# speechbrain/speechbrain

Measured on AMD Instinct MI355X. Metric: audio-sec/s decoded (node), Conformer-L beam=10, higher is better.
Workload: dtype f32

## Files before the change

speechbrain_amd/csrc/hip/sbk_device.h:

```cpp
#pragma once
#include <hip/hip_runtime.h>
#include <stdint.h>

namespace sbk {

constexpr int kWave = 64;

using f32x16 = __attribute__((ext_vector_type(16))) float;
using f32x4 = __attribute__((ext_vector_type(4))) float;

__device__ __forceinline__ f32x16 mfma_32x32x2(float a, float b, f32x16 acc) {
  return __builtin_amdgcn_mfma_f32_32x32x2f32(a, b, acc, 0, 0, 0);
}
__device__ __forceinline__ f32x4 mfma_16x16x4(float a, float b, f32x4 acc) {
  return __builtin_amdgcn_mfma_f32_16x16x4f32(a, b, acc, 0, 0, 0);
}

using bf16x8 = __attribute__((ext_vector_type(8))) __bf16;
__device__ __forceinline__ f32x16 mfma_32x32x16_bf16(bf16x8 a, bf16x8 b, f32x16 acc) {
  return __builtin_amdgcn_mfma_f32_32x32x16_bf16(a, b, acc, 0, 0, 0);
}
__device__ __forceinline__ unsigned short f32_to_bf16(float f) { return __builtin_bit_cast(unsigned short, (__bf16)f); }
__device__ __forceinline__ bf16x8 cvt_bf16x8(const float (&x)[8]) {
  bf16x8 r;
#pragma unroll
  for (int e = 0; e < 8; ++e) r[e] = (__bf16)x[e];
  return r;
}

using u32x4 = __attribute__((ext_vector_type(4))) unsigned;
__device__ __forceinline__ bf16x8 bf16x8_from_words(unsigned w0, unsigned w1, unsigned w2, unsigned w3) {
  u32x4 u = {w0, w1, w2, w3};
  return __builtin_bit_cast(bf16x8, u);
}
using bf16x2 = __attribute__((ext_vector_type(2))) __bf16;
__device__ __forceinline__ unsigned bf16_pair(float x0, float x1) {
  bf16x2 v = {(__bf16)x0, (__bf16)x1};
  return __builtin_bit_cast(unsigned, v);
}

using f16x8 = __attribute__((ext_vector_type(8))) _Float16;
__device__ __forceinline__ f32x16 mfma_32x32x16_f16(f16x8 a, f16x8 b, f32x16 acc) {
  return __builtin_amdgcn_mfma_f32_32x32x16_f16(a, b, acc, 0, 0, 0);
}
__device__ __forceinline__ unsigned short f32_to_f16(float f) { return __builtin_bit_cast(unsigned short, (_Float16)f); }
using fp8x8 = long;
__device__ __forceinline__ f32x16 mfma_32x32x16_fp8(fp8x8 a, fp8x8 b, f32x16 acc) {
  return __builtin_amdgcn_mfma_f32_32x32x16_fp8_fp8(a, b, acc, 0, 0, 0);
}
using i32x8 = __attribute__((ext_vector_type(8))) int;
__device__ __forceinline__ f32x16 mfma_32x32x64_fp8(i32x8 a, i32x8 b, f32x16 acc) {
  return __builtin_amdgcn_mfma_scale_f32_32x32x64_f8f6f4(a, b, acc, 0, 0, 0, 0, 0, 0);
}
__device__ __forceinline__ i32x8 i32x8_from_u4(uint4 lo, uint4 hi) {
  i32x8 r = {(int)lo.x, (int)lo.y, (int)lo.z, (int)lo.w, (int)hi.x, (int)hi.y, (int)hi.z, (int)hi.w};
  return r;
}
__device__ __forceinline__ unsigned short f32x2_to_fp8(float a, float b) {
  a = fminf(fmaxf(a, -448.0f), 448.0f);
  b = fminf(fmaxf(b, -448.0f), 448.0f);
  return (unsigned short)(__builtin_amdgcn_cvt_pk_fp8_f32(a, b, 0, false) & 0xffff);
}

using u16x8 = __attribute__((ext_vector_type(8))) unsigned short;
__device__ __forceinline__ bf16x8 pack_bf16x8(const unsigned short (&h)[8]) {
  u16x8 u;
#pragma unroll
  for (int e = 0; e < 8; ++e) u[e] = h[e];
  return __builtin_bit_cast(bf16x8, u);
}

__device__ __forceinline__ float shfl_xor(float v, int mask) { return __shfl_xor(v, mask, kWave); }
__device__ __forceinline__ int shfl_xor(int v, int mask) { return __shfl_xor(v, mask, kWave); }
__device__ __forceinline__ float shfl(float v, int lane) { return __shfl(v, lane, kWave); }
__device__ __forceinline__ int shfl(int v, int lane) { return __shfl(v, lane, kWave); }

__device__ __forceinline__ void wave_sync() { __builtin_amdgcn_wave_barrier(); }

__device__ __forceinline__ void sched_fence() { __builtin_amdgcn_sched_barrier(0); }

template <int MASK, int SIZE>
__device__ __forceinline__ void sched_group() { __builtin_amdgcn_sched_group_barrier(MASK, SIZE, 0); }

__device__ __forceinline__ void pin(unsigned& x) { asm volatile("" : "+v"(x)); }
__device__ __forceinline__ void pin(float& x) { asm volatile("" : "+v"(x)); }

__device__ __forceinline__ float exp2_raw(float x) { return __builtin_amdgcn_exp2f(x); }
__device__ __forceinline__ bool wave_any(bool p) { return __builtin_amdgcn_ballot_w64(p) != 0; }
__device__ __forceinline__ float gelu_erfc(float x) {
#pragma clang fp contract(off)
  const float z = fabsf(x) * 0.70710678118654752440f;
  const float t = __builtin_amdgcn_rcpf(fmaf(0.3275911f, z, 1.0f));
  float p = fmaf(t, 1.061405429f, -1.453152027f);
  p = fmaf(t, p, 1.421413741f);
  p = fmaf(t, p, -0.284496736f);
  p = fmaf(t, p, 0.254829592f);
  const float q = (p * t) * exp2_raw(-1.44269504088896340736f * (z * z));
  return (0.5f * x) * (x >= 0.0f ? 2.0f - q : q);
}

__device__ __forceinline__ float fast_ldexp(float x, int e) { return __builtin_amdgcn_ldexpf(x, e); }
__device__ __forceinline__ int frexp_exp(float x) { return __builtin_amdgcn_frexp_expf(x); }

template <int CTRL>
__device__ __forceinline__ float dpp_move(float v) {
  return __int_as_float(__builtin_amdgcn_update_dpp(0, __float_as_int(v), CTRL, 0xF, 0xF, true));
}
template <int G>
__device__ __forceinline__ float group_sum(float v) {
  static_assert(G == 1 || G == 2 || G == 4 || G == 8 || G == 16, "group_sum: group width");
  if constexpr (G >= 2) v += dpp_move<0xB1>(v);
  if constexpr (G >= 4) v += dpp_move<0x4E>(v);
  if constexpr (G >= 8) v += dpp_move<0x141>(v);
  if constexpr (G >= 16) v += dpp_move<0x140>(v);
  return v;
}


__device__ __forceinline__ void glds16(const float* src, float* lds_wave_base) {
  const unsigned dst = __builtin_amdgcn_readfirstlane(
      (unsigned)(unsigned long)(__attribute__((address_space(3))) void*)lds_wave_base);
  unsigned keep;
  asm volatile(
      "s_mov_b32 %0, m0\n\ts_mov_b32 m0, %2\n\ts_nop 0\n\tglobal_load_lds_dwordx4 %1, off\n\ts_mov_b32 m0, %0"
      : "=&s"(keep)
      : "v"(src), "s"(dst)
      : "memory");
}
__device__ __forceinline__ void glds16_uniform(const float* base, unsigned lane_byte_offset, float* lds_wave_base) {
  const unsigned dst = __builtin_amdgcn_readfirstlane(
      (unsigned)(unsigned long)(__attribute__((address_space(3))) void*)lds_wave_base);
  unsigned keep;
  asm volatile(
      "s_mov_b32 %0, m0\n\ts_mov_b32 m0, %3\n\ts_nop 0\n\tglobal_load_lds_dwordx4 %1, %2\n\ts_mov_b32 m0, %0"
      : "=&s"(keep)
      : "v"(lane_byte_offset), "s"(base), "s"(dst)
      : "memory");
}
template <bool NT>
__device__ __forceinline__ float4 ld16(const float* p) {
  if constexpr (NT) {
    const f32x4 v = __builtin_nontemporal_load(reinterpret_cast<const f32x4*>(p));
    return make_float4(v[0], v[1], v[2], v[3]);
  } else {
    return *reinterpret_cast<const float4*>(p);
  }
}
template <bool NT>
__device__ __forceinline__ float ld4(const float* p) {
  if constexpr (NT) return __builtin_nontemporal_load(p);
  else return *p;
}
__device__ __forceinline__ int uniform(int v) { return __builtin_amdgcn_readfirstlane(v); }
__device__ __forceinline__ void vm_drain() { asm volatile("s_waitcnt vmcnt(0)" ::: "memory"); }
__device__ __forceinline__ void vm_drain_visible() { __builtin_amdgcn_s_waitcnt(0x0F70); }
template <int N>
__device__ __forceinline__ void vm_wait() {
  static_assert(N >= 0 && N < 64, "vmcnt is a 6-bit counter");
  asm volatile("s_waitcnt vmcnt(%0)" ::"n"(N) : "memory");
}
__device__ __forceinline__ void lds_drain() { asm volatile("s_waitcnt lgkmcnt(0)" ::: "memory"); }
__device__ __forceinline__ void block_barrier_raw() { __builtin_amdgcn_s_barrier(); }
__device__ __forceinline__ void release_agent() {
  __builtin_amdgcn_fence(__ATOMIC_RELEASE, "agent");
  asm volatile("s_waitcnt vmcnt(0)" ::: "memory");
}
__device__ __forceinline__ void acquire_agent() { __builtin_amdgcn_fence(__ATOMIC_ACQUIRE, "agent"); }
__device__ __forceinline__ int atomic_add_agent(int* p, int v) {
// ... 111 lines not shown
```

speechbrain_amd/csrc/relpos_attn.hip:

```cpp
#include "common.h"
#include "internal.h"

namespace {

using sbk::f32x16;

struct AttnArgs {
  const float* qkv;
  const float* pos;
  const float* bias_u;
  const float* bias_v;
  const int32_t* key_len;
  float* out;
  float* attn;
  int B, T, H, SP;
  float scale;
  int chunk, left;
  int out_bf16;
};

__device__ __forceinline__ void key_range(const AttnArgs& a, int i, int klen, int& lo, int& hi) {
  lo = 0;
  hi = klen;
  if (a.chunk > 0) {
    const int c = i / a.chunk;
    hi = min((c + 1) * a.chunk, klen);
    if (a.left >= 0) lo = max(0, (c - a.left) * a.chunk);
  }
}

template <int N>
__device__ __forceinline__ void load_run(float (&dst)[N], const float* __restrict__ p) {
  if constexpr (N % 4 == 0) {
#pragma unroll
    for (int i = 0; i < N / 4; ++i) {
      const float4 v = reinterpret_cast<const float4*>(p)[i];
      dst[4 * i] = v.x; dst[4 * i + 1] = v.y; dst[4 * i + 2] = v.z; dst[4 * i + 3] = v.w;
    }
  } else if constexpr (N % 2 == 0) {
#pragma unroll
    for (int i = 0; i < N / 2; ++i) {
      const float2 v = reinterpret_cast<const float2*>(p)[i];
      dst[2 * i] = v.x; dst[2 * i + 1] = v.y;
    }
  } else {
#pragma unroll
    for (int i = 0; i < N; ++i) dst[i] = p[i];
  }
}

template <int DH, bool ROPE, bool PF, int NW>
__global__ void __launch_bounds__(NW * 64) relpos_attn_kernel(AttnArgs a) {
  constexpr int DH2 = DH / 2;
  constexpr int QP = DH + 1;
  constexpr int NC = (DH + 31) / 32;
  constexpr int NPART = NW / NC;
  constexpr int NT = NW * 64;
  SBK_DYN_LDS(float, lds);
  float* Qu = lds;
  float* Qv = Qu + 32 * QP;
  float* red = Qv + 32 * QP;
  float* S = red + (NW - NC) * 32 * 33;

  const int tid = threadIdx.x, lane = tid & 63, wave = tid >> 6;
  const int jl = lane & 31, half = lane >> 5;
  const int i0 = blockIdx.x * 32, h = blockIdx.y, b = blockIdx.z;
  const int T = a.T, SP = a.SP, d = a.H * DH;
  const size_t row3 = (size_t)3 * d;
  const float* qkv_b = a.qkv + (size_t)b * T * row3 + (size_t)h * 3 * DH;

  for (int idx = tid; idx < 32 * DH; idx += NT) {
    const int i = idx / DH, c = idx % DH;
    const int row = min(i0 + i, T - 1);
    const float q = qkv_b[(size_t)row * row3 + c];
    if constexpr (ROPE) {
      const float qs = qkv_b[(size_t)row * row3 + (c ^ 1)];
      Qu[i * QP + c] = (q * a.pos[(size_t)row * DH + c] + qs * a.bias_u[(size_t)row * DH + c]) * a.scale;
    } else {
      Qu[i * QP + c] = (q + a.bias_u[h * DH + c]) * a.scale;
      Qv[i * QP + c] = (q + a.bias_v[h * DH + c]) * a.scale;
    }
  }
// ... 318 lines not shown
  int kt_begin = 0, kt_end = nkt;
  if (a.chunk > 0) {
    kt_end = min(nkt, ((min(i0 + 31, T - 1) / a.chunk + 1) * a.chunk + 31) / 32);
    if (a.left >= 0) kt_begin = max(0, (i0 / a.chunk - a.left) * a.chunk) / 32;
  }
  float m_run = -INFINITY, l_run = 0.0f;
  f32x16 o[NC];
#pragma unroll
  for (int ct = 0; ct < NC; ++ct)
#pragma unroll
    for (int r = 0; r < 16; ++r) o[ct][r] = 0.0f;

  for (int kt = kt_begin; kt < kt_end; ++kt) {
    const int j0 = kt * 32;
    const int krow = min(j0 + jl, T - 1);
    f32x16 acc;
#pragma unroll
    for (int r = 0; r < 16; ++r) acc[r] = 0.0f;
#pragma unroll
    for (int p = 0; p < 2; ++p) {
      const int c0 = 64 * p + SEG * half;
      float kreg[SEG];
      load_run<SEG>(kreg, qkv_b + ((unsigned)krow * row3u + DH + c0));
      if (rot) rotate_chunks<SEG>(kreg, a.pos + (size_t)krow * DH + c0, a.bias_u + (size_t)krow * DH + c0);
#pragma unroll
      for (int s = 0; s < SEG; ++s) acc = sbk::mfma_32x32x2(kreg[s], qu[p][s], acc);
      sbk::sched_fence();
    }
    auto load_v = [&](int ct, float (&vv)[16]) {
      unsigned t0 = j0 + 4 * half;
      sbk::pin(t0);
#pragma unroll
      for (int r = 0; r < 16; ++r) {
        const unsigned t = min(t0 + (r & 3) + 8 * (r >> 2), (unsigned)(T - 1));
        vv[r] = qkv_b[t * row3u + (2 * DH + ct * 32 + jl)];
      }
    };
    float vv[2][16];
    load_v(0, vv[0]);
    float mx = -INFINITY;
#pragma unroll
    for (int r = 0; r < 16; ++r) {
      const int key = j0 + (r & 3) + 8 * (r >> 2) + 4 * half;
      if (!(key >= lo && key < hi)) acc[r] = -INFINITY;
      mx = fmaxf(mx, acc[r]);
    }
    mx = fmaxf(mx, sbk::shfl_xor(mx, 32));
    const float m_new = fmaxf(m_run, mx);
    const float alpha = m_new == -INFINITY ? 1.0f : expf(m_run - m_new);
    float sum = 0.0f;
#pragma unroll
    for (int r = 0; r < 16; ++r) {
      acc[r] = acc[r] == -INFINITY ? 0.0f : expf(acc[r] - m_new);
      sum += acc[r];
    }
    sum += sbk::shfl_xor(sum, 32);
    l_run = l_run * alpha + sum;
    m_run = m_new;
    if (sbk::wave_any(alpha != 1.0f)) {
#pragma unroll
      for (int ct = 0; ct < NC; ++ct)
#pragma unroll
        for (int r = 0; r < 16; ++r) o[ct][r] *= alpha;
    }
#pragma unroll
    for (int ct = 0; ct < NC; ++ct) {
      if (ct + 1 < NC) load_v(ct + 1, vv[(ct + 1) & 1]);
#pragma unroll
      for (int r = 0; r < 16; ++r) o[ct] = sbk::mfma_32x32x2(vv[ct & 1][r], acc[r], o[ct]);
    }
  }
  if (i0 + jl < T) {
    const float inv = l_run > 0.0f ? 1.0f / l_run : 0.0f;
    float* orow = a.out + ((size_t)b * T + i0 + jl) * d + h * DH;
#pragma unroll
    for (int ct = 0; ct < NC; ++ct)
#pragma unroll
      for (int q = 0; q < 4; ++q)
        *reinterpret_cast<float4*>(orow + ct * 32 + 8 * q + 4 * half) =
            make_float4(o[ct][4 * q] * inv, o[ct][4 * q + 1] * inv, o[ct][4 * q + 2] * inv, o[ct][4 * q + 3] * inv);
  }
}

template <int DH, bool E2 = true>
__global__ void __launch_bounds__(256, 2) relpos_flash_t_kernel(AttnArgs a) {
  constexpr int DH2 = DH / 2;
  constexpr int NC = (DH + 31) / 32;
  __shared__ float Gs[4][64][32];
  const int tid = threadIdx.x, lane = tid & 63, wave = tid >> 6;
  const int jl = lane & 31, half = lane >> 5;
  const int i0 = (blockIdx.x * 4 + wave) * 32, h = blockIdx.y, b = blockIdx.z;
  const int T = a.T, d = a.H * DH;
  if (i0 >= T) return;
  const size_t row3 = (size_t)3 * d;
  const float* qkv_b = a.qkv + (size_t)b * T * row3 + (size_t)h * 3 * DH;
  const int qrow = min(i0 + jl, T - 1);
  float (*G)[32] = Gs[wave];

  float qu[DH2], qv[DH2];
  {
    float qr[DH2], bu[DH2], bv[DH2];
    load_run<DH2>(qr, qkv_b + (size_t)qrow * row3 + half * DH2);
    load_run<DH2>(bu, a.bias_u + h * DH + half * DH2);
    load_run<DH2>(bv, a.bias_v + h * DH + half * DH2);
#pragma unroll
    for (int s = 0; s < DH2; ++s) {
      qu[s] = (qr[s] + bu[s]) * a.scale;
      qv[s] = (qr[s] + bv[s]) * a.scale;
    }
  }
  int klen = T;
  if (a.key_len) klen = min(max(a.key_len[b], 1), T);
  const int nkt = (klen + 31) / 32;
  int lo, hi;
  key_range(a, qrow, klen, lo, hi);
  int kt_begin = 0, kt_end = nkt;
  if (a.chunk > 0) {
    kt_end = min(nkt, ((min(i0 + 31, T - 1) / a.chunk + 1) * a.chunk + 31) / 32);
    if (a.left >= 0) kt_begin = max(0, (i0 / a.chunk - a.left) * a.chunk) / 32;
  }
  float m_run = -INFINITY, l_run = 0.0f;
  f32x16 o[NC];
#pragma unroll
  for (int ct = 0; ct < NC; ++ct)
#pragma unroll
    for (int r = 0; r < 16; ++r) o[ct][r] = 0.0f;

  auto g_block = [&](int first_row, int slot) {
    float preg[DH2];
    const int prow = min(max(first_row + jl, 0), 2 * T - 2);
    load_run<DH2>(preg, a.pos + (size_t)prow * d + h * DH + half * DH2);
    f32x16 g;
#pragma unroll
    for (int r = 0; r < 16; ++r) g[r] = 0.0f;
#pragma unroll
    for (int s = 0; s < DH2; ++s) g = sbk::mfma_32x32x2(preg[s], qv[s], g);
#pragma unroll
    for (int r = 0; r < 16; ++r) G[slot * 32 + (r & 3) + 8 * (r >> 2) + 4 * half][jl] = g[r];
  };
  g_block((T - 1) - i0 - 31 + 32 * kt_begin, kt_begin & 1);
  for (int kt = kt_begin; kt < kt_end; ++kt) {
    const int j0 = kt * 32;
    const int rbase = (T - 1) - i0 - 31 + j0;
    float kreg[DH2];
    load_run<DH2>(kreg, qkv_b + (size_t)min(j0 + jl, T - 1) * row3 + DH + half * DH2);
    f32x16 acc;
#pragma unroll
    for (int r = 0; r < 16; ++r) acc[r] = 0.0f;
#pragma unroll
    for (int s = 0; s < DH2; ++s) acc = sbk::mfma_32x32x2(kreg[s], qu[s], acc);
    g_block(rbase + 32, (kt + 1) & 1);
    float vv[NC][16];
#pragma unroll
    for (int ct = 0; ct < NC; ++ct) {
      const int col = ct * 32 + jl;
      const float* vbase = qkv_b + 2 * DH + (col < DH ? col : 0);
#pragma unroll
      for (int r = 0; r < 16; ++r) {
        const int t = min(j0 + (r & 3) + 8 * (r >> 2) + 4 * half, T - 1);
        vv[ct][r] = col < DH ? vbase[(size_t)t * row3] : 0.0f;
      }
    }
    sbk::wave_sync();
    float mx = -INFINITY;
#pragma unroll
    for (int r = 0; r < 16; ++r) {
      const int jc = (r & 3) + 8 * (r >> 2) + 4 * half;
      const int rr = 31 - jl + jc;
      acc[r] += G[(((kt & 1) + (rr >> 5)) & 1) * 32 + (rr & 31)][jl];
      const int key = j0 + jc;
      if (!(key >= lo && key < hi)) acc[r] = -INFINITY;
      mx = fmaxf(mx, acc[r]);
    }
    sbk::wave_sync();
    mx = fmaxf(mx, sbk::shfl_xor(mx, 32));
    const float m_new = fmaxf(m_run, mx);
    constexpr float kL2E = 1.44269504088896340736f;
    const bool none = m_new == -INFINITY;
    const float nm = none ? 0.0f : -m_new * kL2E;
    float alpha, sum = 0.0f;
    if constexpr (E2) {
      alpha = none ? 1.0f : sbk::exp2_raw(fmaf(m_run, kL2E, nm));
#pragma unroll
      for (int r = 0; r < 16; ++r) {
        acc[r] = none ? 0.0f : sbk::exp2_raw(fmaf(acc[r], kL2E, nm));
        sum += acc[r];
      }
    } else {
      alpha = none ? 1.0f : expf(m_run - m_new);
#pragma unroll
      for (int r = 0; r < 16; ++r) {
        acc[r] = acc[r] == -INFINITY ? 0.0f : expf(acc[r] - m_new);
        sum += acc[r];
      }
    }
    sum += sbk::shfl_xor(sum, 32);
    l_run = l_run * alpha + sum;
    m_run = m_new;
    if (sbk::wave_any(alpha != 1.0f)) {
#pragma unroll
      for (int ct = 0; ct < NC; ++ct)
#pragma unroll
        for (int r = 0; r < 16; ++r) o[ct][r] *= alpha;
    }
#pragma unroll
    for (int r = 0; r < 16; ++r)
#pragma unroll
      for (int ct = 0; ct < NC; ++ct) o[ct] = sbk::mfma_32x32x2(vv[ct][r], acc[r], o[ct]);
  }
  if (i0 + jl < T) {
    const float inv = l_run > 0.0f ? 1.0f / l_run : 0.0f;
    float* orow = a.out + ((size_t)b * T + i0 + jl) * d + h * DH;
#pragma unroll
    for (int ct = 0; ct < NC; ++ct)
#pragma unroll
      for (int r = 0; r < 16; ++r) {
        const int c = ct * 32 + (r & 3) + 8 * (r >> 2) + 4 * half;
        if (c < DH) orow[c] = o[ct][r] * inv;
      }
  }
}

__global__ void __launch_bounds__(256, 2) rope_flash_t_bf16_kernel(AttnArgs a) {
  constexpr int DH = 64;
  using sbk::bf16x8;
  const int tid = threadIdx.x, lane = tid & 63, wave = tid >> 6;
  const int jl = lane & 31, half = lane >> 5;
  const int i0 = (blockIdx.x * 4 + wave) * 32, h = blockIdx.y, b = blockIdx.z;
  const int T = a.T, d = a.H * DH;
  if (i0 >= T) return;
  const size_t row3 = (size_t)3 * d;
  const float* qkv_b = a.qkv + (size_t)b * T * row3 + (size_t)h * 3 * DH;
  const int qrow = min(i0 + jl, T - 1);

  auto load_chunks = [&](const float* row, int frame, float scale, bf16x8 (&dst)[4]) {
#pragma unroll
    for (int t = 0; t < 4; ++t) {
      const int c0 = 16 * t + 8 * half;
      float x[8];
      load_run<8>(x, row + c0);
      if (a.pos != nullptr) {
        float cs[8], sn[8];
        load_run<8>(cs, a.pos + (size_t)frame * DH + c0);
        load_run<8>(sn, a.bias_u + (size_t)frame * DH + c0);
#pragma unroll
        for (int e = 0; e < 8; e += 2) {
          const float x0 = x[e], x1 = x[e + 1];
          x[e] = x0 * cs[e] + x1 * sn[e];
          x[e + 1] = x1 * cs[e + 1] + x0 * sn[e + 1];
        }
      }
#pragma unroll
      for (int e = 0; e < 8; ++e) x[e] *= scale;
      dst[t] = sbk::cvt_bf16x8(x);
    }
  };
  bf16x8 qb[4];
  load_chunks(qkv_b + (size_t)qrow * row3, qrow, a.scale, qb);

  int klen = T;
  if (a.key_len) klen = min(max(a.key_len[b], 1), T);
  const int nkt = (klen + 31) / 32;
  int lo, hi;
  key_range(a, qrow, klen, lo, hi);
  int kt_begin = 0, kt_end = nkt;
  if (a.chunk > 0) {
    kt_end = min(nkt, ((min(i0 + 31, T - 1) / a.chunk + 1) * a.chunk + 31) / 32);
    if (a.left >= 0) kt_begin = max(0, (i0 / a.chunk - a.left) * a.chunk) / 32;
  }
  float m_run = -INFINITY, l_run = 0.0f;
  f32x16 o[2];
#pragma unroll
  for (int ct = 0; ct < 2; ++ct)
#pragma unroll
    for (int r = 0; r < 16; ++r) o[ct][r] = 0.0f;

  for (int kt = kt_begin; kt < kt_end; ++kt) {
    const int j0 = kt * 32;
    bf16x8 kb[4];
    {
      const int krow = min(j0 + jl, T - 1);
      load_chunks(qkv_b + (size_t)krow * row3 + DH, krow, 1.0f, kb);
    }
    f32x16 acc;
#pragma unroll
    for (int r = 0; r < 16; ++r) acc[r] = 0.0f;
#pragma unroll
    for (int t = 0; t < 4; ++t) acc = sbk::mfma_32x32x16_bf16(kb[t], qb[t], acc);
    bf16x8 vb[2][2];
#pragma unroll
    for (int ct = 0; ct < 2; ++ct) {
// ... 155 lines not shown
        acc[u] = sbk::mfma_32x32x16_bf16(kb, qb[t], acc[u]);
      }
    }
    float mx = -INFINITY;
    const bool tail = (kt + 1) * 64 > klen;
    if (tail) {
#pragma unroll
      for (int u = 0; u < 2; ++u)
#pragma unroll
        for (int r = 0; r < 16; ++r)
          if (kt * 64 + 32 * u + 16 * (r >> 3) + 8 * half + (r & 7) >= klen) acc[u][r] = -INFINITY;
    }
#pragma unroll
    for (int u = 0; u < 2; ++u)
#pragma unroll
      for (int r = 0; r < 16; ++r) mx = fmaxf(mx, acc[u][r]);
    mx = fmaxf(mx, sbk::shfl_xor(mx, 32));
    const float m_new = fmaxf(m_run, mx);
    const float c2 = a.scale * 1.44269504088896340736f, mc = -m_new * c2;
    const float alpha = sbk::exp2_raw((m_run - m_new) * c2);
    float sum = 0.0f;
    bf16x8 pb[2][2];
#pragma unroll
    for (int u = 0; u < 2; ++u)
#pragma unroll
      for (int s2 = 0; s2 < 2; ++s2) {
        float x[8];
#pragma unroll
        for (int e = 0; e < 8; ++e) {
          x[e] = sbk::exp2_raw(fmaf(acc[u][8 * s2 + e], c2, mc));
          sum += x[e];
        }
        pb[u][s2] = sbk::cvt_bf16x8(x);
      }
    sum += sbk::shfl_xor(sum, 32);
    l_run = l_run * alpha + sum;
    m_run = m_new;
    if (sbk::wave_any(alpha != 1.0f)) {
#pragma unroll
      for (int c = 0; c < 2; ++c)
#pragma unroll
        for (int r = 0; r < 16; ++r) o[c][r] *= alpha;
    }
#pragma unroll
    for (int u = 0; u < 2; ++u)
#pragma unroll
      for (int s2 = 0; s2 < 2; ++s2)
#pragma unroll
        for (int c = 0; c < 2; ++c) {
          const bf16x8 vb = *reinterpret_cast<const bf16x8*>(Vt + (32 * c + jl) * 32 + (((4 * u + 2 * s2 + half) ^ vsw) << 2));
          o[c] = sbk::mfma_32x32x16_bf16(vb, pb[u][s2], o[c]);
        }
    sbk::vm_drain();
    __syncthreads();
  }
  if (i0 + jl < T) {
    const float inv = 1.0f / l_run;
    unsigned short* orow = a.out + ((size_t)b * T + i0 + jl) * d + h * 64;
#pragma unroll
    for (int c = 0; c < 2; ++c)
#pragma unroll
      for (int q = 0; q < 4; ++q) {
        uint2 pk;
        pk.x = (unsigned)sbk::f32_to_bf16(o[c][4 * q] * inv) | ((unsigned)sbk::f32_to_bf16(o[c][4 * q + 1] * inv) << 16);
        pk.y = (unsigned)sbk::f32_to_bf16(o[c][4 * q + 2] * inv) | ((unsigned)sbk::f32_to_bf16(o[c][4 * q + 3] * inv) << 16);
        *reinterpret_cast<uint2*>(orow + c * 32 + 8 * q + 4 * half) = pk;
      }
  }
}

}
namespace sbk {
int g_attn_exp2 = 1;
}
namespace {
template <int DH, bool ROPE>
int launch_flash(const AttnArgs& a, hipStream_t st) {
  sbk::ProfScope prof(ROPE ? "rope_attention" : "relpos_attention", (ROPE ? 4.0 : 6.0) * a.B * a.H * (double)a.T * a.T * DH,
                      4.0 * a.B * a.T * (4.0 * a.H * DH) + 4.0 * (2.0 * a.T - 1) * a.H * DH, st);
  if constexpr (ROPE) {
    SBK_LAUNCH((rope_flash_t_kernel<DH>), dim3((a.T + 127) / 128, a.H, a.B), dim3(256), 0, st, a);
    return sbk::launch_status("sbk_rope_attention_f32");
  } else {
    if (sbk::g_attn_exp2) {
      SBK_LAUNCH((relpos_flash_t_kernel<DH, true>), dim3((a.T + 127) / 128, a.H, a.B), dim3(256), 0, st, a);
    } else {
      SBK_LAUNCH((relpos_flash_t_kernel<DH, false>), dim3((a.T + 127) / 128, a.H, a.B), dim3(256), 0, st, a);
    }
    return sbk::launch_status("sbk_relpos_attention_f32");
  }
}

int launch_flash128(const AttnArgs& a, hipStream_t st) {
  if (a.attn)
    return sbk::fail(SBK_EINVAL, "rope_attention: the attention-weights output is not instantiated for head_dim 128 (context only)");
  if ((double)a.T * 3.0 * a.H * 128 >= 1073741824.0)
    return sbk::fail(SBK_EINVAL, "rope_attention: head_dim 128 addresses an utterance's rows with 32-bit offsets: T * 3 * d must be < 2^30");
  if (!sbk::aligned16(a.out)) return sbk::fail(SBK_EINVAL, "rope_attention: head_dim 128 writes 16-byte pieces: out must be 16-byte aligned");
  sbk::ProfScope prof("rope_attention", 4.0 * a.B * a.H * (double)a.T * a.T * 128, 4.0 * a.B * a.T * (4.0 * a.H * 128), st);
  SBK_LAUNCH(rope_flash_t128_kernel, dim3((a.T + 127) / 128, a.H, a.B), dim3(256), 0, st, a);
  return sbk::launch_status("sbk_rope_attention_f32");
}

template <int DH, bool ROPE, bool PF, int NW>
int launch_attn_pf(const AttnArgs& a, hipStream_t st);

template <int DH, bool ROPE>
int launch_attn(const AttnArgs& a, hipStream_t st) {
  if (!a.attn) return launch_flash<DH, ROPE>(a, st);
  const size_t lds4 = ((size_t)2 * 32 * (DH + 1) + 3 * 32 * 33 + (size_t)32 * a.SP) * sizeof(float);
  const bool eight = lds4 > 80 * 1024;
  const bool pf = ROPE && eight;
  if (eight) return pf ? launch_attn_pf<DH, ROPE, true, 8>(a, st) : launch_attn_pf<DH, ROPE, false, 8>(a, st);
  return pf ? launch_attn_pf<DH, ROPE, true, 4>(a, st) : launch_attn_pf<DH, ROPE, false, 4>(a, st);
}

template <int DH, bool ROPE, bool PF, int NW>
int launch_attn_pf(const AttnArgs& a, hipStream_t st) {
  constexpr int NCt = (DH + 31) / 32;
  const size_t lds = ((size_t)2 * 32 * (DH + 1) + (NW - NCt) * 32 * 33 + (size_t)32 * a.SP) * sizeof(float);
  if (lds > 160 * 1024) return sbk::fail(SBK_EINVAL, "relpos_attention: T=%d needs %zu B of LDS (max 160 KiB)", a.T, lds);
  if (const int rc = sbk::require_dyn_lds(relpos_attn_kernel<DH, ROPE, PF, NW>, lds, "relpos_attention")) return rc;
  sbk::ProfScope prof(ROPE ? "rope_attention" : "relpos_attention", (ROPE ? 4.0 : 6.0) * a.B * a.H * (double)a.T * a.T * DH,
                      4.0 * a.B * a.T * (4.0 * a.H * DH) + 4.0 * (2.0 * a.T - 1) * a.H * DH, st);
  SBK_LAUNCH((relpos_attn_kernel<DH, ROPE, PF, NW>), dim3((a.T + 31) / 32, a.H, a.B), dim3(NW * 64), lds, st, a);
  return sbk::launch_status(ROPE ? "sbk_rope_attention_f32" : "sbk_relpos_attention_f32");
}

}

namespace sbk {

int relpos_attention(const float* qkv, const float* pos, const float* bias_u, const float* bias_v,
                     const int32_t* key_len, float* out, float* attn, int B, int T, int H, int Dh, float scale,
                     hipStream_t st, int chunk, int left) {
  if (B == 0 || T == 0) return 0;
  const int SP = ((T + 31) / 32) * 32 + 1;
  AttnArgs a{qkv, pos, bias_u, bias_v, key_len, out, attn, B, T, H, SP, scale, chunk, left};
  switch (Dh) {
    case 64: return launch_attn<64, false>(a, st);
    case 36: return launch_attn<36, false>(a, st);
    case 32: return launch_attn<32, false>(a, st);
    case 16: return launch_attn<16, false>(a, st);
    case 8: return launch_attn<8, false>(a, st);
    default: return fail(SBK_EINVAL, "relpos_attention: head_dim %d not instantiated (8,16,32,36,64)", Dh);
  }
}

int rope_attention(const float* qkv, const float* cosines, const float* sines, const int32_t* key_len, float* out,
                   float* attn, int B, int T, int H, int Dh, float scale, hipStream_t st, int chunk, int left) {
  if (B == 0 || T == 0) return 0;
  const int SP = ((T + 31) / 32) * 32 + 1;
  AttnArgs a{qkv, cosines, sines, nullptr, key_len, out, attn, B, T, H, SP, scale, chunk, left};
  switch (Dh) {
    case 128: return launch_flash128(a, st);
    case 64: return launch_attn<64, true>(a, st);
    case 36: return launch_attn<36, true>(a, st);
    case 32: return launch_attn<32, true>(a, st);
    case 16: return launch_attn<16, true>(a, st);
    case 8: return launch_attn<8, true>(a, st);
    default: return fail(SBK_EINVAL, "rope_attention: head_dim %d not instantiated (8,16,32,36,64,128)", Dh);
  }
}
}

extern "C" int sbk_rope_attention_f32(const float* qkv, const float* cosines, const float* sines,
                                      const int32_t* key_len, float* out, float* attn, int B, int T, int H, int Dh,
                                      int table_rows, float scale, int chunk_size, int left_chunks,
                                      sbk_stream_t stream) {
  if (B == 0 || T == 0) return 0;
// ... 81 lines not shown
```

speechbrain_amd/native.py:

```python

from __future__ import annotations

import collections
import contextlib
import ctypes
import math
import os
import threading
import weakref
from ctypes import POINTER, c_char_p, c_float, c_int, c_int32, c_void_p
from typing import Optional

import torch

_HERE = os.path.dirname(os.path.abspath(__file__))
LIB_PATH = os.path.join(_HERE, "csrc", "libsbk_hip.so")

ACT_NONE, ACT_SWISH, ACT_GELU, ACT_RELU, ACT_LEAKY_RELU = 0, 1, 2, 3, 4

_lib = None


class SbkError(RuntimeError):
    pass
# ... 161 lines not shown
        "sbk_w2v_utt_norm_f32": ([p, p, i, ctypes.c_long, f, p], c_int),
        "sbk_wavlm_attention_max_frames": ([], c_int),
        "sbk_wavlm_attention_f32": ([p, p, p, p, p, p, p, p, i, i, i, i, f, p], c_int),
        "sbk_hypermix_split_frames": ([], c_int),
        "sbk_hypermix_workspace_bytes": ([i, i, i, i], ctypes.c_size_t),
        "sbk_hypermix_f32": ([p] * 13 + [f, p, p, p, ctypes.c_size_t, i, i, i, i, i, p], c_int),
        "sbk_rnn_layer_route": ([i, i, i, i], c_int),
        "sbk_rnn_layer_f32": ([p] * 9 + [i] * 6 + [p], c_int),
        "sbk_crdnn_conv1_f32": ([p] * 6 + [i, i, i, i, f, f, p], c_int),
        "sbk_crdnn_im2col_f32": ([p, p, i, i, i, i, i, i, p], c_int),
        "sbk_crdnn_norm_pool_f32": ([p] * 4 + [i] * 6 + [f, f, p], c_int),
        "sbk_layernorm_f32": ([p, p, p, p, i, i, f, i, p], c_int),
        "sbk_log_softmax_f32": ([p, p, i, i, f, f, p], c_int),
        "sbk_ctc_greedy_decode_f32": ([p, p, p, p, i, i, i, i, p], c_int),
        "sbk_ctc_beam_search_workspace_bytes": ([i, i, i, i, i], ctypes.c_size_t),
        "sbk_ctc_beam_search_f32": ([p, p, p, i, POINTER(CTCBeamConfig), p, ctypes.c_size_t, p, p, p, i, i, i, p], c_int),
        "sbk_ctc_beam_search_lm_f32": ([p, p, p, i, POINTER(CTCBeamConfig), POINTER(CTCLMTables), p, ctypes.c_size_t, p, p, p,
                                        p, i, i, i, p], c_int),
        "sbk_transducer_greedy_f32": ([POINTER(TransducerWeights), POINTER(TransducerConfig), p, p, p, p, p, p, p, i, i, p],
                                      c_int),
        "sbk_lstm_f32": ([p, p, p, p, p, p, p, i, i, i, p], c_int),
        "sbk_transducer_beam_workspace_bytes": ([POINTER(TransducerWeights), POINTER(TransducerBeamConfig), i, i],
                                                ctypes.c_size_t),
        "sbk_transducer_beam_search_f32": ([POINTER(TransducerWeights), POINTER(TransducerBeamConfig), p, p, ctypes.c_size_t,
                                            p, p, p, p, p, i, i, p], c_int),
        "sbk_transducer_beam_lm_workspace_bytes": ([POINTER(TransducerWeights), POINTER(RNNLMWeights),
                                                    POINTER(TransducerBeamConfig), i, i], ctypes.c_size_t),
        "sbk_transducer_beam_search_lm_f32": ([POINTER(TransducerWeights), POINTER(RNNLMWeights), f,
                                               POINTER(TransducerBeamConfig), p, p, ctypes.c_size_t, p, p, p, p, p, i, i, p],
                                              c_int),
        "sbk_beam_search_workspace_bytes": ([POINTER(DecoderWeights), POINTER(SearchConfig), i, i], ctypes.c_size_t),
        "sbk_beam_search_f32": ([POINTER(DecoderWeights), POINTER(SearchConfig), p, p, p, p, p, ctypes.c_size_t, p, p,
                                 p, p, p, p, p, POINTER(c_int32), i, i, p], c_int),
        "sbk_greedy_search_workspace_bytes": ([POINTER(DecoderWeights), i, i, i], ctypes.c_size_t),
        "sbk_greedy_search_f32": ([POINTER(DecoderWeights), p, p, p, ctypes.c_size_t, p, p, p, POINTER(c_int32), i, i,
                                   i, i, i, i, i, p], c_int),
        "sbk_prompted_greedy_search_workspace_bytes": ([POINTER(DecoderWeights), i, i, i, i], ctypes.c_size_t),
        "sbk_prompted_greedy_search_f32": ([POINTER(DecoderWeights), p, p, p, i, p, p, p, ctypes.c_size_t, p, p, i, i, p, p,
                                            POINTER(c_int32), i, i, i, i, i, p], c_int),
        "sbk_decoder_prefix_workspace_bytes": ([POINTER(DecoderWeights), i, i, i], ctypes.c_size_t),
        "sbk_decoder_prefix_f32": ([POINTER(DecoderWeights), p, p, p, p, ctypes.c_size_t, p, i, i, i, p], c_int),
        "sbk_lm_prefix_workspace_bytes": ([POINTER(LMWeights), i, i], ctypes.c_size_t),
        "sbk_lm_prefix_f32": ([POINTER(LMWeights), p, p, ctypes.c_size_t, p, i, i, p], c_int),
    }
    for name, (args, res) in sig.items():
        fn = getattr(lib, name)
        fn.argtypes = args
        fn.restype = res
    return sig


EXPORTS: tuple = ()
_LIBS: dict = {}


def load(path: Optional[str] = None):
    global _lib, EXPORTS
    if _lib is not None and path is None:
        return _lib
    path = path or LIB_PATH
    if path not in _LIBS:
        if not os.path.exists(path):
            raise SbkError(
                f"{path} is missing: the MI355X kernels are not built. Run `python -m speechbrain_amd.csrc.build` "
                "(hipcc, gfx950). There is no CPU fallback."
            )
        lib = ctypes.CDLL(path)
        exports = tuple(_declare(lib).keys())
        if lib.sbk_abi_version() != 11:
            raise SbkError(f"ABI version mismatch: {lib.sbk_abi_version()}")
        _LIBS[path] = (lib, exports)
    _lib, EXPORTS = _LIBS[path]
    return _lib


KNOBS = {
    "skinny_off": 2, "cross_rows": 4, "cross_fc256": 8, "tiled_splitk": 14, "sk_mode": 18, "sk_min_rows": 24,
    "x3_route_rows": 34, "x3_route_tiles": 35, "score_fused": 40, "x3r_mode": 41, "x3r_min_rows": 42, "x3r_ln": 45,
    "persist": 47, "persist_grid": 48, "persist_stamps": 49, "x3r_xc": 51, "nt_mask": 53, "self_anc": 55, "x3r_pair": 58,
    "persist_tree": 59, "attn_exp2": 60, "lp256": 61, "x3p_fast_epi": 63,
}


@contextlib.contextmanager
def knobs(**values):
    lib = load()
    wanted = {KNOBS[name]: int(value) for name, value in values.items()}
    found = {key: lib.sbk_prof_get_knob(key) for key in wanted}
    try:
        for key, value in wanted.items():
            lib.sbk_prof_set_knob(key, value)
        yield
    finally:
        for key, value in found.items():
            lib.sbk_prof_set_knob(key, value)


def _chk(rc: int, what: str):
    if rc != 0:
        raise SbkError(f"{what} failed (rc={rc}): {_lib.sbk_last_error().decode()}")


def _dev_ok(*ts):
    for t in ts:
        if t is None:
            continue
        if not t.is_cuda:
            raise SbkError(
                "speechbrain_amd ops run on an MI355X (HIP) device only; got a CPU tensor. "
                "Move the module and inputs to 'cuda' (there is no CPU fallback)."
            )
        if not t.is_contiguous():
            raise SbkError("non-contiguous tensor passed to a kernel")


def _p(t: Optional[torch.Tensor]):
    return None if t is None else c_void_p(t.data_ptr())


_STREAM_WS = {}
_STREAM_WS_LOCK = threading.RLock()
_STREAM_WS_REFS = {}


def _ws_key(stream):
    return (id(load()), stream.device.index, stream.cuda_stream) if stream is not None else (id(load()), "host", 0)


def retain_stream_workspace(stream):
    key = _ws_key(stream)
    with _STREAM_WS_LOCK:
        _STREAM_WS_REFS[key] = _STREAM_WS_REFS.get(key, 0) + 1


class _Workspace:
    __slots__ = ("buf", "off", "ptr", "key")

    def __init__(self, nbytes, device, align=256, floor=0, per_stream=False):
        size = max(nbytes, floor) + align
        self.buf, self.key = (_search_workspace(size, device) if per_stream
                              else (torch.empty(size, dtype=torch.uint8, device=device), None))
        self.off = (-self.buf.data_ptr()) % align
        self.ptr = c_void_p(self.buf.data_ptr() + self.off)

    def __enter__(self):
        return self

    def __exit__(self, *exc):
        _search_workspace_done(self.key)


def _register_workspace(key, device, handle):
    lib = load()
    with _STREAM_WS_LOCK:
        if key in _STREAM_WS:
            return
        nbytes = lib.sbk_stream_workspace_bytes()
        ws = _Workspace(nbytes, device)
        ctx = torch.cuda.device(device) if getattr(device, "type", None) == "cuda" else contextlib.nullcontext()
        with ctx:
            _chk(lib.sbk_stream_workspace_set(c_void_p(handle) if handle is not None else None, ws.ptr, nbytes),
                 "sbk_stream_workspace_set")
        _STREAM_WS[key] = ws


def forget_stream_owner(stream):
    key = _ws_key(stream)
    with _STREAM_WS_LOCK:
        left = _STREAM_WS_REFS.get(key, 0) - 1
        if left > 0:
            _STREAM_WS_REFS[key] = left
# ... 1615 lines not shown
```

Before: 13140.

## Prefetch next K and position rows one tile ahead in relpos flash attention

Restructures the relpos flash-attention tile loop so the K and positional-embedding rows for the next key tile are loaded while the current tile computes. The loop is software-pipelined with scheduling fences and register pins. It also switches address arithmetic to 32-bit offsets and simplifies the G-ring index and the key-mask comparisons, which cuts per-element integer work. The new path is on by default, guarded by a size check, and can be disabled through a bit in the attn_exp2 knob. The cost is extra register pressure from double-buffered K and P registers, which could hurt occupancy at launch bounds of 256 threads with 2 blocks.

New measurement: 13250, median of 6. About the same (+0.8%).

```diff
diff --git a/speechbrain_amd/csrc/hip/sbk_device.h b/speechbrain_amd/csrc/hip/sbk_device.h
--- a/speechbrain_amd/csrc/hip/sbk_device.h
+++ b/speechbrain_amd/csrc/hip/sbk_device.h
@@ -84,6 +84,7 @@
 
 __device__ __forceinline__ void pin(unsigned& x) { asm volatile("" : "+v"(x)); }
 __device__ __forceinline__ void pin(float& x) { asm volatile("" : "+v"(x)); }
+__device__ __forceinline__ void pin(f32x4& x) { asm volatile("" : "+v"(x)); }
 
 __device__ __forceinline__ float exp2_raw(float x) { return __builtin_amdgcn_exp2f(x); }
 __device__ __forceinline__ bool wave_any(bool p) { return __builtin_amdgcn_ballot_w64(p) != 0; }
diff --git a/speechbrain_amd/csrc/relpos_attn.hip b/speechbrain_amd/csrc/relpos_attn.hip
--- a/speechbrain_amd/csrc/relpos_attn.hip
+++ b/speechbrain_amd/csrc/relpos_attn.hip
@@ -1,3 +1,5 @@
+#include <type_traits>
+
 #include "common.h"
 #include "internal.h"
 
@@ -482,12 +484,31 @@
   }
 }
 
-template <int DH, bool E2 = true>
+__device__ __forceinline__ const float* at32(const float* base, unsigned elem) {
+  return reinterpret_cast<const float*>(reinterpret_cast<const char*>(base) + elem * 4u);
+}
+template <int N>
+__device__ __forceinline__ void pin_run(float (&x)[N]) {
+  if constexpr (N % 4 == 0) {
+#pragma unroll
+    for (int i = 0; i < N / 4; ++i) {
+      sbk::f32x4 t;
+      t[0] = x[4 * i]; t[1] = x[4 * i + 1]; t[2] = x[4 * i + 2]; t[3] = x[4 * i + 3];
+      sbk::pin(t);
+      x[4 * i] = t[0]; x[4 * i + 1] = t[1]; x[4 * i + 2] = t[2]; x[4 * i + 3] = t[3];
+    }
+  } else {
+#pragma unroll
+    for (int s = 0; s < N; ++s) sbk::pin(x[s]);
+  }
+}
+
+template <int DH, bool E2 = true, bool AH = true>
 __global__ void __launch_bounds__(256, 2) relpos_flash_t_kernel(AttnArgs a) {
   constexpr int DH2 = DH / 2;
   constexpr int NC = (DH + 31) / 32;
   __shared__ float Gs[4][64][32];
-  const int tid = threadIdx.x, lane = tid & 63, wave = tid >> 6;
+  const int tid = threadIdx.x, lane = tid & 63, wave = AH ? sbk::uniform(tid >> 6) : tid >> 6;
   const int jl = lane & 31, half = lane >> 5;
   const int i0 = (blockIdx.x * 4 + wave) * 32, h = blockIdx.y, b = blockIdx.z;
   const int T = a.T, d = a.H * DH;
@@ -526,10 +547,44 @@
 #pragma unroll
     for (int r = 0; r < 16; ++r) o[ct][r] = 0.0f;
 
-  auto g_block = [&](int first_row, int slot) {
-    float preg[DH2];
+  float kreg[DH2], preg[DH2], vv[NC][16];
+  const unsigned row3u = 3u * (unsigned)d;
+  auto k_req = [&](int kt) SBK_INLINE_LAMBDA {
+    if constexpr (AH) load_run<DH2>(kreg, at32(qkv_b, (unsigned)min(kt * 32 + jl, T - 1) * row3u + (unsigned)(DH + half * DH2)));
+    else load_run<DH2>(kreg, qkv_b + (size_t)min(kt * 32 + jl, T - 1) * row3 + DH + half * DH2);
+  };
+  auto p_req = [&](int first_row) SBK_INLINE_LAMBDA {
     const int prow = min(max(first_row + jl, 0), 2 * T - 2);
-    load_run<DH2>(preg, a.pos + (size_t)prow * d + h * DH + half * DH2);
+    if constexpr (AH) load_run<DH2>(preg, at32(a.pos + h * DH, (unsigned)prow * (unsigned)d + (unsigned)(half * DH2)));
+    else load_run<DH2>(preg, a.pos + (size_t)prow * d + h * DH + half * DH2);
+  };
+  auto v_req = [&](int kt) SBK_INLINE_LAMBDA {
+    if constexpr (AH) {
+#pragma unroll
+      for (int r = 0; r < 16; ++r) {
+        const int t = min(kt * 32 + (r & 3) + 8 * (r >> 2) + 4 * half, T - 1);
+#pragma unroll
+        for (int ct = 0; ct < NC; ++ct) {
+          const int col = ct * 32 + jl;
+          vv[ct][r] = col < DH ? *at32(qkv_b + 2 * DH, (unsigned)t * row3u + (unsigned)(col < DH ? col : 0)) : 0.0f;
+        }
+        sbk::sched_fence();
+      }
+    } else {
+#pragma unroll
+      for (int ct = 0; ct < NC; ++ct) {
+        const int col = ct * 32 + jl;
+        const float* vbase = qkv_b + 2 * DH + (col < DH ? col : 0);
+#pragma unroll
+        for (int r = 0; r < 16; ++r) {
+          const int t = min(kt * 32 + (r & 3) + 8 * (r >> 2) + 4 * half, T - 1);
+          vv[ct][r] = col < DH ? vbase[(size_t)t * row3] : 0.0f;
+        }
+      }
+    }
+  };
+  auto g_chain = [&](int slot) SBK_INLINE_LAMBDA {
+    if constexpr (AH) pin_run(preg);
     f32x16 g;
 #pragma unroll
     for (int r = 0; r < 16; ++r) g[r] = 0.0f;
@@ -538,38 +593,65 @@
 #pragma unroll
     for (int r = 0; r < 16; ++r) G[slot * 32 + (r & 3) + 8 * (r >> 2) + 4 * half][jl] = g[r];
   };
-  g_block((T - 1) - i0 - 31 + 32 * kt_begin, kt_begin & 1);
-  for (int kt = kt_begin; kt < kt_end; ++kt) {
+  const int first = (T - 1) - i0 - 31 + 32 * kt_begin;
+  if constexpr (AH) {
+    if (kt_begin < kt_end) {
+      p_req(first);
+      k_req(kt_begin);
+      sbk::sched_fence();
+      g_chain(kt_begin & 1);
+      sbk::sched_fence();
+      p_req(first + 32);
+      sbk::sched_fence();
+    }
+  } else {
+    p_req(first);
+    g_chain(kt_begin & 1);
+  }
+  auto tile = [&](int kt, auto more_c) SBK_INLINE_LAMBDA {
+    constexpr bool MORE = decltype(more_c)::value;
     const int j0 = kt * 32;
     const int rbase = (T - 1) - i0 - 31 + j0;
-    float kreg[DH2];
-    load_run<DH2>(kreg, qkv_b + (size_t)min(j0 + jl, T - 1) * row3 + DH + half * DH2);
+    if constexpr (AH) pin_run(kreg);
+    else k_req(kt);
     f32x16 acc;
 #pragma unroll
     for (int r = 0; r < 16; ++r) acc[r] = 0.0f;
 #pragma unroll
     for (int s = 0; s < DH2; ++s) acc = sbk::mfma_32x32x2(kreg[s], qu[s], acc);
-    g_block(rbase + 32, (kt + 1) & 1);
-    float vv[NC][16];
-#pragma unroll
-    for (int ct = 0; ct < NC; ++ct) {
-      const int col = ct * 32 + jl;
-      const float* vbase = qkv_b + 2 * DH + (col < DH ? col : 0);
-#pragma unroll
-      for (int r = 0; r < 16; ++r) {
-        const int t = min(j0 + (r & 3) + 8 * (r >> 2) + 4 * half, T - 1);
-        vv[ct][r] = col < DH ? vbase[(size_t)t * row3] : 0.0f;
-      }
+    if constexpr (AH) {
+      sbk::sched_fence();
+      if constexpr (MORE) k_req(kt + 1);
+      v_req(kt);
+      sbk::sched_fence();
+    } else {
+      p_req(rbase + 32);
+    }
+    g_chain((kt + 1) & 1);
+    if constexpr (AH) {
+      sbk::sched_fence();
+      if constexpr (MORE) p_req(rbase + 64);
+      sbk::sched_fence();
+    } else {
+      v_req(kt);
     }
     sbk::wave_sync();
     float mx = -INFINITY;
+    unsigned ring0 = (unsigned)((kt & 1) * 32 + 31 - jl + 4 * half);
+    if constexpr (AH) sbk::pin(ring0);
+    const int klo = lo - (j0 + 4 * half), khi = hi - (j0 + 4 * half);
 #pragma unroll
     for (int r = 0; r < 16; ++r) {
       const int jc = (r & 3) + 8 * (r >> 2) + 4 * half;
       const int rr = 31 - jl + jc;
-      acc[r] += G[(((kt & 1) + (rr >> 5)) & 1) * 32 + (rr & 31)][jl];
+      if constexpr (AH) acc[r] += G[(ring0 + (r & 3) + 8 * (r >> 2)) & 63][jl];
+      else acc[r] += G[(((kt & 1) + (rr >> 5)) & 1) * 32 + (rr & 31)][jl];
       const int key = j0 + jc;
-      if (!(key >= lo && key < hi)) acc[r] = -INFINITY;
+      if constexpr (AH) {
+        if (!((r & 3) + 8 * (r >> 2) >= klo && (r & 3) + 8 * (r >> 2) < khi)) acc[r] = -INFINITY;
+      } else {
+        if (!(key >= lo && key < hi)) acc[r] = -INFINITY;
+      }
       mx = fmaxf(mx, acc[r]);
     }
     sbk::wave_sync();
@@ -603,10 +685,25 @@
 #pragma unroll
         for (int r = 0; r < 16; ++r) o[ct][r] *= alpha;
     }
+    if constexpr (AH) {
+#pragma unroll
+      for (int ct = 0; ct < NC; ++ct)
+#pragma unroll
+        for (int r = 0; r < 16; ++r) sbk::pin(vv[ct][r]);
+    }
 #pragma unroll
     for (int r = 0; r < 16; ++r)
 #pragma unroll
       for (int ct = 0; ct < NC; ++ct) o[ct] = sbk::mfma_32x32x2(vv[ct][r], acc[r], o[ct]);
+  };
+  if constexpr (AH) {
+    if (kt_begin < kt_end) {
+      int kt = kt_begin;
+      for (; kt + 1 < kt_end; ++kt) tile(kt, std::true_type{});
+      tile(kt, std::false_type{});
+    }
+  } else {
+    for (int kt = kt_begin; kt < kt_end; ++kt) tile(kt, std::false_type{});
   }
   if (i0 + jl < T) {
     const float inv = l_run > 0.0f ? 1.0f / l_run : 0.0f;
@@ -928,10 +1025,17 @@
     SBK_LAUNCH((rope_flash_t_kernel<DH>), dim3((a.T + 127) / 128, a.H, a.B), dim3(256), 0, st, a);
     return sbk::launch_status("sbk_rope_attention_f32");
   } else {
-    if (sbk::g_attn_exp2) {
-      SBK_LAUNCH((relpos_flash_t_kernel<DH, true>), dim3((a.T + 127) / 128, a.H, a.B), dim3(256), 0, st, a);
+    const dim3 grid((a.T + 127) / 128, a.H, a.B);
+    const bool exp2 = (sbk::g_attn_exp2 & 1) != 0;
+    const bool ahead = !(sbk::g_attn_exp2 & 2) && (double)a.T * 3.0 * a.H * DH < 1073741824.0;
+    if (ahead && exp2) {
+      SBK_LAUNCH((relpos_flash_t_kernel<DH, true, true>), grid, dim3(256), 0, st, a);
+    } else if (ahead) {
+      SBK_LAUNCH((relpos_flash_t_kernel<DH, false, true>), grid, dim3(256), 0, st, a);
+    } else if (exp2) {
+      SBK_LAUNCH((relpos_flash_t_kernel<DH, true, false>), grid, dim3(256), 0, st, a);
     } else {
-      SBK_LAUNCH((relpos_flash_t_kernel<DH, false>), dim3((a.T + 127) / 128, a.H, a.B), dim3(256), 0, st, a);
+      SBK_LAUNCH((relpos_flash_t_kernel<DH, false, false>), grid, dim3(256), 0, st, a);
     }
     return sbk::launch_status("sbk_relpos_attention_f32");
   }
diff --git a/speechbrain_amd/native.py b/speechbrain_amd/native.py
--- a/speechbrain_amd/native.py
+++ b/speechbrain_amd/native.py
@@ -267,11 +267,21 @@
 }
 
 
+KNOB_FLAGS = {"attn_exp2": (60, 1, 1), "attn_ahead": (60, 2, 0)}
+
+
 @contextlib.contextmanager
 def knobs(**values):
     lib = load()
-    wanted = {KNOBS[name]: int(value) for name, value in values.items()}
-    found = {key: lib.sbk_prof_get_knob(key) for key in wanted}
+    keys = {KNOB_FLAGS[name][0] if name in KNOB_FLAGS else KNOBS[name] for name in values}
+    found = {key: lib.sbk_prof_get_knob(key) for key in keys}
+    wanted = dict(found)
+    for name, value in values.items():
+        if name in KNOB_FLAGS:
+            key, mask, sets = KNOB_FLAGS[name]
+            wanted[key] = wanted[key] | mask if bool(int(value)) == bool(sets) else wanted[key] & ~mask
+        else:
+            wanted[KNOBS[name]] = int(value)
     try:
         for key, value in wanted.items():
             lib.sbk_prof_set_knob(key, value)
```
